# TencentARC/SEED-Story

Measured on AMD Instinct MI355X. Metric: story-steps/sec (text + 1024x1024 image), higher is better.
Workload: dtype bf16

## Files before the change

seed-story_amd/csrc/ss_attn.hip:

```cpp
#include "ss_common.h"

namespace ss {

struct AttnArgs {
    const void *q, *k, *v;
    void* out;
    int q_len, kv_len, hd, n_heads;
    int64_t q_sb, q_sh, q_ss, k_sb, k_sh, k_ss, v_sb, v_sh, v_ss, o_sb, o_sh, o_ss;
    float scale;
    int causal_br;
    int xcd_heads;
    int ragged;
    int kv_len_b[8];
};

template <typename T> struct AttnMma;
template <> struct AttnMma<bf16_t> {
    static __device__ __forceinline__ f32x4_t run(const uint4& a, const uint4& b, f32x4_t c) {
        return __builtin_amdgcn_mfma_f32_16x16x32_bf16(__builtin_bit_cast(bf16x8_t, a),
                                                       __builtin_bit_cast(bf16x8_t, b), c, 0, 0, 0);
    }
};
template <> struct AttnMma<f16_t> {
    static __device__ __forceinline__ f32x4_t run(const uint4& a, const uint4& b, f32x4_t c) {
// ... 311 lines not shown
                    }
            } else {
#pragma unroll
                for (int kb = 0; kb < NKB; ++kb)
#pragma unroll
                    for (int r = 0; r < 4; ++r) tmax = fmaxf(tmax, s[qb][kb][r]);
            }
            tmax = fmaxf(tmax, __shfl_xor(tmax, 16, 64));
            tmax = fmaxf(tmax, __shfl_xor(tmax, 32, 64));
            const float m_new = fmaxf(m_run[qb], tmax);
            const float alpha = __builtin_amdgcn_exp2f((m_run[qb] - m_new) * sl2);
            const float nm = -fmaxf(m_new, -1e29f) * sl2;
            float lsum = 0.f;
#pragma unroll
            for (int kb = 0; kb < NKB; ++kb)
#pragma unroll
                for (int r = 0; r < 4; ++r) {
                    const float p = __builtin_amdgcn_exp2f(fmaf(s[qb][kb][r], sl2, nm));
                    s[qb][kb][r] = p;
                    lsum += p;
                }
            lsum += __shfl_xor(lsum, 16, 64);
            lsum += __shfl_xor(lsum, 32, 64);
            l_run[qb] = l_run[qb] * alpha + lsum;
            m_run[qb] = m_new;
#pragma unroll
            for (int i = 0; i < NDB; ++i)
#pragma unroll
                for (int r = 0; r < 4; ++r) o[qb][i][r] *= alpha;
#pragma unroll
            for (int kp2 = 0; kp2 < NKB / 2; ++kp2) {
                float pf[8];
#pragma unroll
                for (int r = 0; r < 4; ++r) { pf[r] = s[qb][2 * kp2][r]; pf[4 + r] = s[qb][2 * kp2 + 1][r]; }
                pfrag[qb][kp2] = pack<T>(pf);
            }
        }
#pragma unroll
        for (int kp2 = 0; kp2 < NKB / 2; ++kp2) {
#pragma unroll
            for (int db = 0; db < NDB; ++db) {
                const int kr0 = (2 * kp2) * 16 + grp * 4 + (l15 >> 2);
                const int dcol = db * 16 + (l15 & 3) * 4;
                const v4s_t v0 = __builtin_amdgcn_ds_read_tr16_b64_v4i16((lds_v4s_t*)(Vb + kr0 * ROWB + dcol * 2));
                const v4s_t v1 = __builtin_amdgcn_ds_read_tr16_b64_v4i16((lds_v4s_t*)(Vb + (kr0 + 16) * ROWB + dcol * 2));
                const uint2 w0 = __builtin_bit_cast(uint2, v0), w1 = __builtin_bit_cast(uint2, v1);
                const uint4 vfrag = make_uint4(w0.x, w0.y, w1.x, w1.y);
                o[0][db] = AttnMma<T>::run(vfrag, pfrag[0][kp2], o[0][db]);
                o[1][db] = AttnMma<T>::run(vfrag, pfrag[1][kp2], o[1][db]);
            }
        }
    }

#pragma unroll
    for (int qb = 0; qb < 2; ++qb) {
        if (qi[qb] >= a.q_len) continue;
        const float inv = l_run[qb] > 0.f ? 1.0f / l_run[qb] : 0.f;
        T* op = (T*)a.out + (int64_t)b * a.o_sb + (int64_t)h * a.o_sh + (int64_t)qi[qb] * a.o_ss;
#pragma unroll
        for (int db = 0; db < NDB; ++db) {
            const int d = db * 16 + grp * 4;
            if (d + 3 < hd && ((a.o_ss | a.o_sh | a.o_sb) & 3) == 0) {
                float pk[8] = {o[qb][db][0] * inv, o[qb][db][1] * inv, o[qb][db][2] * inv, o[qb][db][3] * inv, 0, 0, 0, 0};
                const uint4 u = pack<T>(pk);
                *reinterpret_cast<uint2*>(op + d) = make_uint2(u.x, u.y);
            } else {
#pragma unroll
                for (int r = 0; r < 4; ++r)
                    if (d + r < hd) Tr<T>::st(op + d + r, o[qb][db][r] * inv);
            }
        }
    }
}
#endif

__device__ __forceinline__ float max3_asm(float a, float b, float c) {
    float r;
    asm("v_max3_f32 %0, %1, %2, %3" : "=v"(r) : "v"(a), "v"(b), "v"(c));
    return r;
}
template <typename T> struct OnesFrag;
template <> struct OnesFrag<bf16_t> { static constexpr uint32_t kPair = 0x3F803F80u; };
template <> struct OnesFrag<f16_t> { static constexpr uint32_t kPair = 0x3C003C00u; };
__device__ __forceinline__ void attn_block_of_grid(const AttnArgs& a, int& bh, int& qblk) {
    if (gridDim.y == 1 && a.xcd_heads > 0) {
        const int id = blockIdx.x, xcd = id & 7, j = id >> 3;
        const int nqb = a.xcd_heads;
        bh = (j / nqb) * 8 + xcd;
        qblk = j - (j / nqb) * nqb;
    } else {
        bh = blockIdx.y; qblk = blockIdx.x;
    }
}

template <typename T, int HD>
__device__ __forceinline__ void flash_compute_s(const char* Kb, int l15, int grp, const uint4 (&qf)[2][HD / 32],
                                                f32x4_t (&s)[2][kBKV / 16]) {
    constexpr int CPR = HD / 8, ROWB = HD * 2;
#pragma unroll
    for (int kb = 0; kb < kBKV / 16; ++kb) {
        s[0][kb] = f32x4_t{0.f, 0.f, 0.f, 0.f};
        s[1][kb] = f32x4_t{0.f, 0.f, 0.f, 0.f};
        const int r = kb * 16 + l15;
#pragma unroll
        for (int ks = 0; ks < HD / 32; ++ks) {
            const uint4 kf = *reinterpret_cast<const uint4*>(Kb + r * ROWB + (((ks * 4 + grp) ^ (r & (CPR - 1))) << 4));
            s[0][kb] = AttnMma<T>::run(kf, qf[0][ks], s[0][kb]);
            s[1][kb] = AttnMma<T>::run(kf, qf[1][ks], s[1][kb]);
        }
    }
}

template <typename T, int HD, bool VSWZ>
__global__ __launch_bounds__(256) __attribute__((amdgpu_waves_per_eu(HD <= 64 ? 3 : 2)))
void flash_attn3_kernel(const AttnArgs a) {
    constexpr int V = 8;
    constexpr int BQ2 = 128;
    constexpr int CPR = HD / V;
    constexpr int KPI = 64 / CPR;
    constexpr int NI = kBKV / KPI;
    constexpr int IPW = NI / 4;
    constexpr int ROWB = HD * 2;
    constexpr int TILE_B = kBKV * ROWB;
    constexpr int NDB = HD / 16, NKB = kBKV / 16, NKS = HD / 32;
    constexpr float THR_L2 = 8.0f;
    extern __shared__ __attribute__((aligned(16))) char smem_raw[];

    const int tid = threadIdx.x, lane = tid & 63;
    const int wid = __builtin_amdgcn_readfirstlane(tid >> 6);
    const int l15 = lane & 15, grp = lane >> 4;
    int bh, qblk;
    attn_block_of_grid(a, bh, qblk);
    const int b = bh / a.n_heads, h = bh % a.n_heads;
    const int kvl = a.ragged ? a.kv_len_b[b] : a.kv_len;
    const int q0 = qblk * BQ2;
    const int hd = a.hd;
    const T* __restrict__ qp = (const T*)a.q + (int64_t)b * a.q_sb + (int64_t)h * a.q_sh;
    const T* __restrict__ kp = (const T*)a.k + (int64_t)b * a.k_sb + (int64_t)h * a.k_sh;
    const T* __restrict__ vp = (const T*)a.v + (int64_t)b * a.v_sb + (int64_t)h * a.v_sh;
    const int shift = kvl - a.q_len;
    const T* zero = reinterpret_cast<const T*>(g_attn_zero_page);
    const uint32_t lds0 = __builtin_amdgcn_readfirstlane((uint32_t)(size_t)(lds_void2_t*)smem_raw);
    const float sl2 = a.scale * 1.4426950408889634f;
    const float thr_raw = THR_L2 / fmaxf(sl2, 1e-30f);

    int qi[2];
    uint4 qf[2][NKS];
#pragma unroll
    for (int qb = 0; qb < 2; ++qb) {
        qi[qb] = q0 + wid * 32 + qb * 16 + l15;
#pragma unroll
        for (int ks = 0; ks < NKS; ++ks) {
            const int d = ks * 32 + grp * 8;
            qf[qb][ks] = (qi[qb] < a.q_len && d < hd) ? ld16(qp + (int64_t)qi[qb] * a.q_ss + d) : make_uint4(0, 0, 0, 0);
        }
    }
    f32x4_t o[2][NDB], osum[2];
#pragma unroll
    for (int qb = 0; qb < 2; ++qb) {
        osum[qb] = f32x4_t{0.f, 0.f, 0.f, 0.f};
#pragma unroll
        for (int i = 0; i < NDB; ++i) o[qb][i] = f32x4_t{0.f, 0.f, 0.f, 0.f};
    }
    float m_run[2] = {-1e30f, -1e30f};
    const uint4 ones = make_uint4(OnesFrag<T>::kPair, OnesFrag<T>::kPair, OnesFrag<T>::kPair, OnesFrag<T>::kPair);

// ... 62 lines not shown
#pragma unroll
                for (int kb = 0; kb < NKB; ++kb)
#pragma unroll
                    for (int r = 0; r < 4; ++r) {
                        const int kg = t0 + kb * 16 + grp * 4 + r;
                        const bool ok = kg < kvl && (!a.causal_br || kg <= qi[qb] + shift);
                        s[qb][kb][r] = ok ? s[qb][kb][r] : -1e30f;
                    }
            }
            float tmax;
            asm volatile("s_nop 7\n\ts_nop 7\n\tv_max3_f32 %0, %1, %2, %3"
                         : "=v"(tmax) : "v"(s[qb][0][0]), "v"(s[qb][0][1]), "v"(s[qb][0][2]));
            tmax = max3_asm(tmax, s[qb][0][3], s[qb][1][0]);
#pragma unroll
            for (int kb = 1; kb < NKB; ++kb) {
                tmax = max3_asm(tmax, s[qb][kb][1], s[qb][kb][2]);
                if (kb + 1 < NKB) tmax = max3_asm(tmax, s[qb][kb][3], s[qb][kb + 1][0]);
                else tmax = max3_asm(tmax, s[qb][kb][3], s[qb][kb][3]);
            }
            if (__any(tmax > m_run[qb] + thr_raw)) {
                tmax = fmaxf(tmax, __shfl_xor(tmax, 16, 64));
                tmax = fmaxf(tmax, __shfl_xor(tmax, 32, 64));
                const float m_new = fmaxf(m_run[qb], tmax);
                const float alpha = __builtin_amdgcn_exp2f((m_run[qb] - m_new) * sl2);
                m_run[qb] = m_new;
#pragma unroll
                for (int i = 0; i < NDB; ++i)
#pragma unroll
                    for (int r = 0; r < 4; ++r) o[qb][i][r] *= alpha;
#pragma unroll
                for (int r = 0; r < 4; ++r) osum[qb][r] *= alpha;
            }
            const float nm = -fmaxf(m_run[qb], -1e29f) * sl2;
#pragma unroll
            for (int kp2 = 0; kp2 < NKB / 2; ++kp2) {
                float pf[8];
#pragma unroll
                for (int r = 0; r < 4; ++r) {
                    pf[r] = __builtin_amdgcn_exp2f(fmaf(s[qb][2 * kp2][r], sl2, nm));
                    pf[4 + r] = __builtin_amdgcn_exp2f(fmaf(s[qb][2 * kp2 + 1][r], sl2, nm));
                }
                pfrag[qb][kp2] = pack<T>(pf);
            }
        }
#pragma unroll
        for (int kp2 = 0; kp2 < NKB / 2; ++kp2) {
            osum[0] = AttnMma<T>::run(ones, pfrag[0][kp2], osum[0]);
            osum[1] = AttnMma<T>::run(ones, pfrag[1][kp2], osum[1]);
#pragma unroll
            for (int db = 0; db < NDB; ++db) {
                const char* vb = Vb + voff[db] + kp2 * 32 * ROWB;
                const v4s_t v0 = __builtin_amdgcn_ds_read_tr16_b64_v4i16((lds_v4s_t*)(vb));
                const v4s_t v1 = __builtin_amdgcn_ds_read_tr16_b64_v4i16((lds_v4s_t*)(vb + 16 * ROWB));
                const uint2 w0 = __builtin_bit_cast(uint2, v0), w1 = __builtin_bit_cast(uint2, v1);
                const uint4 vfrag = make_uint4(w0.x, w0.y, w1.x, w1.y);
                o[0][db] = AttnMma<T>::run(vfrag, pfrag[0][kp2], o[0][db]);
                o[1][db] = AttnMma<T>::run(vfrag, pfrag[1][kp2], o[1][db]);
            }
        }
    }

#pragma unroll
    for (int qb = 0; qb < 2; ++qb) {
        if (qi[qb] >= a.q_len) continue;
        const float l = osum[qb][0];
        const float inv = l > 0.f ? 1.0f / l : 0.f;
        T* op = (T*)a.out + (int64_t)b * a.o_sb + (int64_t)h * a.o_sh + (int64_t)qi[qb] * a.o_ss;
#pragma unroll
        for (int db = 0; db < NDB; ++db) {
            const int d = db * 16 + grp * 4;
            if (d + 3 < hd && ((a.o_ss | a.o_sh | a.o_sb) & 3) == 0) {
                float pk[8] = {o[qb][db][0] * inv, o[qb][db][1] * inv, o[qb][db][2] * inv, o[qb][db][3] * inv, 0, 0, 0, 0};
                const uint4 u = pack<T>(pk);
                *reinterpret_cast<uint2*>(op + d) = make_uint2(u.x, u.y);
            } else {
#pragma unroll
                for (int r = 0; r < 4; ++r)
                    if (d + r < hd) Tr<T>::st(op + d + r, o[qb][db][r] * inv);
            }
        }
    }
}

template <typename T, int HD, bool PIPE, int NW = 4>
__global__ __launch_bounds__(64 * NW) __attribute__((amdgpu_waves_per_eu(PIPE ? 2 : (NW >= 8 ? 4 : 3))))
void flash_attn3p_kernel(const AttnArgs a) {
    static_assert(HD == 64, "v3p: head_dim <= 64");
    static_assert(NW == 4 || NW == 8 || NW == 16, "waves per workgroup");
    constexpr int V = 8;
    constexpr int BQ2 = 32 * NW;
    constexpr int CPR = HD / V;
    constexpr int KPI = 64 / CPR;
    constexpr int NI = kBKV / KPI;
    constexpr int IPW = NI / NW > 0 ? NI / NW : 1;
    constexpr int ROWB = HD * 2;
    constexpr int TILE_B = kBKV * ROWB;
    constexpr int NDB = HD / 16, NKB = kBKV / 16, NKS = HD / 32;
    constexpr int NSTAGE = 3;
    constexpr float THR_L2 = 8.0f;
    extern __shared__ __attribute__((aligned(16))) char smem_raw[];

    const int tid = threadIdx.x, lane = tid & 63;
    const int wid = __builtin_amdgcn_readfirstlane(tid >> 6);
    const int l15 = lane & 15, grp = lane >> 4;
    int bh, qblk;
    attn_block_of_grid(a, bh, qblk);
    const int b = bh / a.n_heads, h = bh % a.n_heads;
    const int kvl = a.ragged ? a.kv_len_b[b] : a.kv_len;
    const int q0 = qblk * BQ2;
    const int hd = a.hd;
    const T* __restrict__ qp = (const T*)a.q + (int64_t)b * a.q_sb + (int64_t)h * a.q_sh;
    const T* __restrict__ kp = (const T*)a.k + (int64_t)b * a.k_sb + (int64_t)h * a.k_sh;
    const T* __restrict__ vp = (const T*)a.v + (int64_t)b * a.v_sb + (int64_t)h * a.v_sh;
    const int shift = kvl - a.q_len;
    const T* zero = reinterpret_cast<const T*>(g_attn_zero_page);
    const uint32_t lds0 = __builtin_amdgcn_readfirstlane((uint32_t)(size_t)(lds_void2_t*)smem_raw);
    const float sl2 = a.scale * 1.4426950408889634f;
    const float thr_raw = THR_L2 / fmaxf(sl2, 1e-30f);

    int qi[2];
    uint4 qf[2][NKS];
#pragma unroll
    for (int qb = 0; qb < 2; ++qb) {
        qi[qb] = q0 + wid * 32 + qb * 16 + l15;
#pragma unroll
        for (int ks = 0; ks < NKS; ++ks) {
            const int d = ks * 32 + grp * 8;
            qf[qb][ks] = (qi[qb] < a.q_len && d < hd) ? ld16(qp + (int64_t)qi[qb] * a.q_ss + d) : make_uint4(0, 0, 0, 0);
        }
    }
    f32x4_t o[2][NDB], osum[2];
#pragma unroll
    for (int qb = 0; qb < 2; ++qb) {
        osum[qb] = f32x4_t{0.f, 0.f, 0.f, 0.f};
#pragma unroll
        for (int i = 0; i < NDB; ++i) o[qb][i] = f32x4_t{0.f, 0.f, 0.f, 0.f};
    }
    float m_run[2] = {-1e30f, -1e30f};
    const uint4 ones = make_uint4(OnesFrag<T>::kPair, OnesFrag<T>::kPair, OnesFrag<T>::kPair, OnesFrag<T>::kPair);

    int kv_end = kvl;
    if (a.causal_br) {
        const int lim = q0 + BQ2 - 1 + shift + 1;
        if (lim < kv_end) kv_end = lim;
        if (kv_end < 0) kv_end = 0;
    }
    const int ntiles = (kv_end + kBKV - 1) / kBKV;
    if (ntiles == 0) {
#pragma unroll
        for (int qb = 0; qb < 2; ++qb) {
            if (qi[qb] >= a.q_len) continue;
            T* op = (T*)a.out + (int64_t)b * a.o_sb + (int64_t)h * a.o_sh + (int64_t)qi[qb] * a.o_ss;
#pragma unroll
            for (int db = 0; db < NDB; ++db)
#pragma unroll
                for (int r = 0; r < 4; ++r) {
                    const int d = db * 16 + grp * 4 + r;
                    if (d < hd) Tr<T>::st(op + d, 0.f);
                }
        }
        return;
    }

    auto vsw = [](int r) { return (r >> 1) & 3; };

    const int skey = lane / CPR, spc = lane % CPR;
    int dkey[IPW];
    const T* kbase_l[IPW];
    const T* vbase_l[IPW];
// ... 26 lines not shown
            attn_dma16(vs, __builtin_amdgcn_readfirstlane(vbase + roff));
        }
    };

    const int vrow = grp * 4 + (l15 >> 2);
    uint32_t voff[NDB];
#pragma unroll
    for (int db = 0; db < NDB; ++db) voff[db] = (uint32_t)(vrow * ROWB + ((db ^ vsw(vrow)) << 5) + (l15 & 3) * 8);

    auto compute_s = [&](int slot, f32x4_t (&s)[2][NKB]) {
        const char* Kb = smem_raw + slot * 2 * TILE_B;
        flash_compute_s<T, HD>(Kb, l15, grp, qf, s);
    };

    auto softmax_pv = [&](int t, int slot, f32x4_t (&s)[2][NKB]) {
        const char* Vb = smem_raw + slot * 2 * TILE_B + TILE_B;
        const int t0 = t * kBKV;
        uint4 pfrag[2][NKB / 2];
        const bool need_mask = a.causal_br || (t0 + kBKV > kvl);
#pragma unroll
        for (int qb = 0; qb < 2; ++qb) {
            if (need_mask) {
#pragma unroll
                for (int kb = 0; kb < NKB; ++kb)
#pragma unroll
                    for (int r = 0; r < 4; ++r) {
                        const int kg = t0 + kb * 16 + grp * 4 + r;
                        const bool ok = kg < kvl && (!a.causal_br || kg <= qi[qb] + shift);
                        s[qb][kb][r] = ok ? s[qb][kb][r] : -1e30f;
                    }
            }
            float tmax;
            asm volatile("s_nop 7\n\ts_nop 7\n\tv_max3_f32 %0, %1, %2, %3"
                         : "=v"(tmax) : "v"(s[qb][0][0]), "v"(s[qb][0][1]), "v"(s[qb][0][2]));
            tmax = max3_asm(tmax, s[qb][0][3], s[qb][1][0]);
#pragma unroll
            for (int kb = 1; kb < NKB; ++kb) {
                tmax = max3_asm(tmax, s[qb][kb][1], s[qb][kb][2]);
                if (kb + 1 < NKB) tmax = max3_asm(tmax, s[qb][kb][3], s[qb][kb + 1][0]);
                else tmax = max3_asm(tmax, s[qb][kb][3], s[qb][kb][3]);
            }
            if (__any(tmax > m_run[qb] + thr_raw)) {
                tmax = fmaxf(tmax, __shfl_xor(tmax, 16, 64));
                tmax = fmaxf(tmax, __shfl_xor(tmax, 32, 64));
                const float m_new = fmaxf(m_run[qb], tmax);
                const float alpha = __builtin_amdgcn_exp2f((m_run[qb] - m_new) * sl2);
                m_run[qb] = m_new;
#pragma unroll
                for (int i = 0; i < NDB; ++i)
#pragma unroll
                    for (int r = 0; r < 4; ++r) o[qb][i][r] *= alpha;
#pragma unroll
                for (int r = 0; r < 4; ++r) osum[qb][r] *= alpha;
            }
            const float nm = -fmaxf(m_run[qb], -1e29f) * sl2;
#pragma unroll
            for (int kp2 = 0; kp2 < NKB / 2; ++kp2) {
                float pf[8];
#pragma unroll
                for (int r = 0; r < 4; ++r) {
                    pf[r] = __builtin_amdgcn_exp2f(fmaf(s[qb][2 * kp2][r], sl2, nm));
                    pf[4 + r] = __builtin_amdgcn_exp2f(fmaf(s[qb][2 * kp2 + 1][r], sl2, nm));
                }
                pfrag[qb][kp2] = pack<T>(pf);
            }
        }
#pragma unroll
        for (int kp2 = 0; kp2 < NKB / 2; ++kp2) {
            osum[0] = AttnMma<T>::run(ones, pfrag[0][kp2], osum[0]);
            osum[1] = AttnMma<T>::run(ones, pfrag[1][kp2], osum[1]);
#pragma unroll
            for (int db = 0; db < NDB; ++db) {
                const char* vb = Vb + voff[db] + kp2 * 32 * ROWB;
                const v4s_t v0 = __builtin_amdgcn_ds_read_tr16_b64_v4i16((lds_v4s_t*)(vb));
                const v4s_t v1 = __builtin_amdgcn_ds_read_tr16_b64_v4i16((lds_v4s_t*)(vb + 16 * ROWB));
                const uint2 w0 = __builtin_bit_cast(uint2, v0), w1 = __builtin_bit_cast(uint2, v1);
                const uint4 vfrag = make_uint4(w0.x, w0.y, w1.x, w1.y);
                o[0][db] = AttnMma<T>::run(vfrag, pfrag[0][kp2], o[0][db]);
                o[1][db] = AttnMma<T>::run(vfrag, pfrag[1][kp2], o[1][db]);
            }
        }
    };

    if constexpr (!PIPE) {
        issue_tile(0, 0);
        if (1 < ntiles) issue_tile(1, 1);
        int stage = 0;
        f32x4_t sc[2][NKB];
        for (int t = 0; t < ntiles; ++t) {
            if (t + 1 < ntiles) asm volatile("s_waitcnt vmcnt(%0)" ::"n"(2 * IPW) : "memory");
            else asm volatile("s_waitcnt vmcnt(0)" ::: "memory");
            __syncthreads();
            if (t + NSTAGE - 1 < ntiles) {
                int ns = stage + NSTAGE - 1;
                if (ns >= NSTAGE) ns -= NSTAGE;
                issue_tile(t + NSTAGE - 1, ns);
            }
            compute_s(stage, sc);
            softmax_pv(t, stage, sc);
            if (++stage == NSTAGE) stage = 0;
        }
    } else {
    issue_tile(0, 0);
    if (1 < ntiles) issue_tile(1, 1);
    if (1 < ntiles) asm volatile("s_waitcnt vmcnt(%0)" ::"n"(2 * IPW) : "memory");
    else asm volatile("s_waitcnt vmcnt(0)" ::: "memory");
    __syncthreads();
    f32x4_t sA[2][NKB], sB[2][NKB];
    compute_s(0, sA);

    auto iteration = [&](int t, int slot, f32x4_t (&cur)[2][NKB], f32x4_t (&nxt)[2][NKB]) {
        const bool more = t + 1 < ntiles;
        int s1 = slot + 1; if (s1 >= NSTAGE) s1 -= NSTAGE;
        int s2 = s1 + 1;   if (s2 >= NSTAGE) s2 -= NSTAGE;
        if (more) {
            asm volatile("s_waitcnt vmcnt(0)" ::: "memory");
            __syncthreads();
            if (t + 2 < ntiles) issue_tile(t + 2, s2);
            compute_s(s1, nxt);
        }
        softmax_pv(t, slot, cur);
    };
    int t = 0, slot = 0;
    while (true) {
        iteration(t, slot, sA, sB);
        if (++t >= ntiles) break;
        if (++slot == NSTAGE) slot = 0;
        iteration(t, slot, sB, sA);
        if (++t >= ntiles) break;
        if (++slot == NSTAGE) slot = 0;
    }
    }

#pragma unroll
    for (int qb = 0; qb < 2; ++qb) {
        if (qi[qb] >= a.q_len) continue;
        const float l = osum[qb][0];
        const float inv = l > 0.f ? 1.0f / l : 0.f;
        T* op = (T*)a.out + (int64_t)b * a.o_sb + (int64_t)h * a.o_sh + (int64_t)qi[qb] * a.o_ss;
#pragma unroll
        for (int db = 0; db < NDB; ++db) {
            const int d = db * 16 + grp * 4;
            if (d + 3 < hd && ((a.o_ss | a.o_sh | a.o_sb) & 3) == 0) {
                float pk[8] = {o[qb][db][0] * inv, o[qb][db][1] * inv, o[qb][db][2] * inv, o[qb][db][3] * inv, 0, 0, 0, 0};
                const uint4 u = pack<T>(pk);
                *reinterpret_cast<uint2*>(op + d) = make_uint2(u.x, u.y);
            } else {
#pragma unroll
                for (int r = 0; r < 4; ++r)
                    if (d + r < hd) Tr<T>::st(op + d + r, o[qb][db][r] * inv);
            }
        }
    }
}

#if SS_EXPERIMENTAL
template <typename T>
__global__ __launch_bounds__(256) __attribute__((amdgpu_waves_per_eu(2)))
void cross_attn64_kernel(const AttnArgs a, int n_items, int items_per_block, int chunks_per_pair) {
    constexpr int HD = 64, NDB = 4, NKB = 4, NKS = 2;
    const int tid = threadIdx.x, lane = tid & 63;
    const int wid = __builtin_amdgcn_readfirstlane(tid >> 6);
    const int l15 = lane & 15, grp = lane >> 4;
    const float sl2 = a.scale * 1.4426950408889634f;
    const uint4 ones = make_uint4(OnesFrag<T>::kPair, OnesFrag<T>::kPair, OnesFrag<T>::kPair, OnesFrag<T>::kPair);
    const int kvl = a.kv_len;
    const bool o_vec = ((a.o_ss | a.o_sh | a.o_sb) & 3) == 0;
    int it = blockIdx.x * items_per_block;
    int it_end = it + items_per_block;
    if (it_end > n_items) it_end = n_items;
    if (it >= it_end) return;

    uint4 kf[NKB][NKS];
    uint4 vf[NKB / 2][NDB];
    int cur_pair = -1;
    auto load_q = [&](int item, uint4 (&qf)[2][NKS]) {
        const int pair = item / chunks_per_pair, chunk = item - pair * chunks_per_pair;
        const int b = pair / a.n_heads, h = pair - b * a.n_heads;
        const T* __restrict__ qp = (const T*)a.q + (int64_t)b * a.q_sb + (int64_t)h * a.q_sh;
#pragma unroll
        for (int qb = 0; qb < 2; ++qb) {
            const int qi = chunk * 128 + wid * 32 + qb * 16 + l15;
// ... 72 lines not shown
                    pf[r] = __builtin_amdgcn_exp2f(fmaf(s[qb][2 * kp2][r], sl2, nm));
                    pf[4 + r] = __builtin_amdgcn_exp2f(fmaf(s[qb][2 * kp2 + 1][r], sl2, nm));
                }
                pfrag[qb][kp2] = pack<T>(pf);
            }
        }
        f32x4_t o[2][NDB], osum[2];
#pragma unroll
        for (int qb = 0; qb < 2; ++qb) {
            osum[qb] = f32x4_t{0.f, 0.f, 0.f, 0.f};
#pragma unroll
            for (int i = 0; i < NDB; ++i) o[qb][i] = f32x4_t{0.f, 0.f, 0.f, 0.f};
        }
#pragma unroll
        for (int kp2 = 0; kp2 < NKB / 2; ++kp2) {
            osum[0] = AttnMma<T>::run(ones, pfrag[0][kp2], osum[0]);
            osum[1] = AttnMma<T>::run(ones, pfrag[1][kp2], osum[1]);
#pragma unroll
            for (int db = 0; db < NDB; ++db) {
                o[0][db] = AttnMma<T>::run(vf[kp2][db], pfrag[0][kp2], o[0][db]);
                o[1][db] = AttnMma<T>::run(vf[kp2][db], pfrag[1][kp2], o[1][db]);
            }
        }
#pragma unroll
        for (int qb = 0; qb < 2; ++qb) {
            const int qi = chunk * 128 + wid * 32 + qb * 16 + l15;
            if (qi >= a.q_len) continue;
            const float l = osum[qb][0];
            const float inv = l > 0.f ? 1.0f / l : 0.f;
            T* op = (T*)a.out + (int64_t)b * a.o_sb + (int64_t)h * a.o_sh + (int64_t)qi * a.o_ss;
#pragma unroll
            for (int db = 0; db < NDB; ++db) {
                const int d = db * 16 + grp * 4;
                if (o_vec) {
                    float pk[8] = {o[qb][db][0] * inv, o[qb][db][1] * inv, o[qb][db][2] * inv, o[qb][db][3] * inv, 0, 0, 0, 0};
                    const uint4 u = pack<T>(pk);
                    *reinterpret_cast<uint2*>(op + d) = make_uint2(u.x, u.y);
                } else {
#pragma unroll
                    for (int r = 0; r < 4; ++r) Tr<T>::st(op + d + r, o[qb][db][r] * inv);
                }
            }
        }
        if (more) {
#pragma unroll
            for (int qb = 0; qb < 2; ++qb)
#pragma unroll
                for (int ks = 0; ks < NKS; ++ks) qf[qb][ks] = qn[qb][ks];
        }
    }
}

template <typename T>
static int cross_attn64_launch(const AttnArgs& a, int64_t batch, hipStream_t s) {
    const int cpp = cdiv(a.q_len, 128);
    const int64_t n_items = batch * a.n_heads * cpp;
    static int n_cu = 0;
    if (n_cu == 0) {
        int dev = 0;
        hipDeviceProp_t p;
        if (hipGetDevice(&dev) == hipSuccess && hipGetDeviceProperties(&p, dev) == hipSuccess) n_cu = p.multiProcessorCount;
        if (n_cu <= 0) n_cu = 256;
    }
    const int64_t max_blocks = (int64_t)2 * n_cu;
    const int ipb = (int)((n_items + max_blocks - 1) / max_blocks);
    const int grid = (int)((n_items + ipb - 1) / ipb);
    hipLaunchKernelGGL((cross_attn64_kernel<T>), dim3((unsigned)grid), dim3(256), 0, s, a, (int)n_items, ipb, cpp);
    SS_LAUNCH_CHECK("cross_attn64");
    return SS_OK;
}

#endif

static dim3 flash_grid(AttnArgs& a, int nqb, int64_t bh) {
    a.xcd_heads = 0;
    if (bh % 8 == 0 && nqb > 1 && knob(K_attn_xcd)) {
        a.xcd_heads = nqb;
        return dim3((unsigned)(nqb * bh), 1);
    }
    return dim3((unsigned)nqb, (unsigned)bh);
}

template <typename T, bool PIPE>
static int flash3p_launch(const AttnArgs& a, int64_t batch, hipStream_t s) {
    const int64_t kv_tiles = a.ragged ? 3 : cdiv(a.kv_len, kBKV);
    const size_t lds = (size_t)(kv_tiles < 3 && !PIPE ? (kv_tiles < 1 ? 1 : kv_tiles) : 3) * 2 * kBKV * 64 * 2;
    const int64_t bh = batch * a.n_heads;
    const int aw = knob(K_attn_waves);
    const bool many = a.ragged || a.kv_len >= 512;
    const bool w16 = !PIPE && (aw == 16 || (aw == 0 && many && a.q_len >= 2048 && (int64_t)cdiv(a.q_len, 512) * bh >= 1024));
    const bool w8 = !PIPE && !w16 && (aw == 8 || (aw == 0 && many && a.q_len >= 512 && (int64_t)cdiv(a.q_len, 256) * bh >= 1024));
    const int nqb = cdiv(a.q_len, w16 ? 512 : w8 ? 256 : 128);
    AttnArgs a2 = a;
    const dim3 grid = flash_grid(a2, nqb, bh);
    if constexpr (!PIPE) {
        if (w16) {
            hipLaunchKernelGGL((flash_attn3p_kernel<T, 64, false, 16>), grid, dim3(1024), lds, s, a2);
            SS_LAUNCH_CHECK("flash_attn3p");
            return SS_OK;
        }
        if (w8) {
            hipLaunchKernelGGL((flash_attn3p_kernel<T, 64, false, 8>), grid, dim3(512), lds, s, a2);
            SS_LAUNCH_CHECK("flash_attn3p");
            return SS_OK;
        }
    }
    hipLaunchKernelGGL((flash_attn3p_kernel<T, 64, PIPE>), grid, dim3(256), lds, s, a2);
    SS_LAUNCH_CHECK("flash_attn3p");
    return SS_OK;
}

template <typename T, int HD, bool VSWZ>
static int flash3_launch_hd(const AttnArgs& a, int64_t batch, hipStream_t s) {
    const size_t lds = (size_t)(HD <= 64 ? 3 : 2) * 2 * kBKV * HD * 2;
    const int nqb = cdiv(a.q_len, 128);
    const int64_t bh = batch * a.n_heads;
    AttnArgs a2 = a;
    const dim3 grid = flash_grid(a2, nqb, bh);
    hipLaunchKernelGGL((flash_attn3_kernel<T, HD, VSWZ>), grid, dim3(256), lds, s, a2);
    SS_LAUNCH_CHECK("flash_attn3");
    return SS_OK;
}

#if SS_EXPERIMENTAL
template <typename T, int HD>
static int flash2_launch_hd(const AttnArgs& a, int64_t batch, hipStream_t s) {
    const size_t lds = (size_t)(HD <= 64 ? 3 : 2) * 2 * kBKV * HD * 2;
    dim3 grid((unsigned)cdiv(a.q_len, 128), (unsigned)(batch * a.n_heads));
    hipLaunchKernelGGL((flash_attn2_kernel<T, HD>), grid, dim3(256), lds, s, a);
    SS_LAUNCH_CHECK("flash_attn2");
    return SS_OK;
}
#endif

template <typename T, int HD>
static int flash_launch_hd(const AttnArgs& a, int64_t batch, hipStream_t s) {
    constexpr int V = Tr<T>::kVec;
    const size_t lds = ((size_t)kBKV * (HD + V) + (size_t)HD * (kBKV + V)) * sizeof(T);
    dim3 grid((unsigned)cdiv(a.q_len, kBQ), (unsigned)(batch * a.n_heads));
    hipLaunchKernelGGL((flash_attn_kernel<T, HD>), grid, dim3(256), lds, s, a);
    SS_LAUNCH_CHECK("flash_attn");
    return SS_OK;
}

template <typename T>
int attention_launch(const AttnArgs& a, int64_t batch, hipStream_t s) {
    constexpr int V = Tr<T>::kVec;
    SS_REQUIRE(a.hd % V == 0 && a.hd > 0 && a.hd <= 128, "attention: head_dim %d unsupported", a.hd);
    SS_REQUIRE(a.q_ss % V == 0 && a.k_ss % V == 0 && a.v_ss % V == 0 && a.q_sh % V == 0 && a.k_sh % V == 0 &&
                   a.v_sh % V == 0 && a.q_sb % V == 0 && a.k_sb % V == 0 && a.v_sb % V == 0,
               "attention: strides must be multiples of %d elements", V);
    SS_REQUIRE(!a.causal_br || a.kv_len >= a.q_len, "attention: causal needs kv_len >= q_len");
    if (a.q_len == 0 || batch == 0) return SS_OK;
    SS_REQUIRE(a.kv_len > 0, "attention: kv_len == 0");
    if constexpr (V == 8) {
        const int ver = knob(K_attn_ver);
#if SS_EXPERIMENTAL
        if (a.hd == 64 && a.kv_len <= 64 && !a.causal_br && !a.ragged && a.q_len >= 128 && ver >= 3 && knob(K_attn_cross64))
            return cross_attn64_launch<T>(a, batch, s);
#endif
        if (ver == 5 && a.q_len >= 32 && a.hd <= 64) return flash3p_launch<T, true>(a, batch, s);
        if (ver == 6 && a.q_len >= 32 && a.hd <= 64) return flash3p_launch<T, false>(a, batch, s);
        if (ver >= 3 && a.q_len >= 32) {
            if (ver == 3 || ver >= 5) {
                if (a.hd <= 64) return flash3_launch_hd<T, 64, true>(a, batch, s);
                return flash3_launch_hd<T, 128, true>(a, batch, s);
            }
            if (a.hd <= 64) return flash3_launch_hd<T, 64, false>(a, batch, s);
            return flash3_launch_hd<T, 128, false>(a, batch, s);
        }
#if SS_EXPERIMENTAL
        if (ver == 2 && a.q_len >= 32) {
            if (a.hd <= 64) return flash2_launch_hd<T, 64>(a, batch, s);
            return flash2_launch_hd<T, 128>(a, batch, s);
        }
#else
        SS_REQUIRE(ver != 2, "attention: attn_ver 2 (flash v2) is only in the EXPERIMENTAL=1 build");
#endif
    }
    if (a.hd <= 64) return flash_launch_hd<T, 64>(a, batch, s);
    return flash_launch_hd<T, 128>(a, batch, s);
}

int attention_dev(const AttnArgs& a, int64_t batch, int dtype, hipStream_t s) {
    return SS_DISPATCH(dtype, attention_launch, a, batch, s);
}

struct DecodeArgs {
    const void* q;
    const void* qkv_raw;
    void *kc, *vc;
    const void *cos_t, *sin_t;
    float* part;
    const int32_t* kv_len_dev;
    const int32_t* pos_dev;
    const int32_t* done_flag;
    int hd, n_heads, cap, nsplit;
    float scale;
    int nb, state_stride;
    int64_t q_stride, cache_stride, part_stride, out_stride;
};

template <typename T>
__global__ __launch_bounds__(256) void attn_decode_kernel(const DecodeArgs a0) {
    DecodeArgs a = a0;
    {
        const int b = blockIdx.z;
        const int64_t so = (int64_t)b * a.state_stride;
        if (a.done_flag) a.done_flag += so;
        a.kv_len_dev += so;
        if (a.pos_dev) a.pos_dev += so;
        if (a.q) a.q = (const T*)a.q + b * a.q_stride;
        if (a.qkv_raw) a.qkv_raw = (const T*)a.qkv_raw + b * a.q_stride;
        a.kc = (T*)a.kc + b * a.cache_stride;
        a.vc = (T*)a.vc + b * a.cache_stride;
        a.part += b * a.part_stride;
    }
    constexpr int V = Tr<T>::kVec;
    constexpr int KPT = 4;
    extern __shared__ __attribute__((aligned(16))) char smem_raw[];
    float* sm = reinterpret_cast<float*>(smem_raw);
    if (a.done_flag && *a.done_flag) return;
    const int h = blockIdx.x, sp = blockIdx.y, tid = threadIdx.x;
    const int hd = a.hd;
    const int LPK = hd / V, NKG = 256 / LPK;
    const int kg = tid / LPK, dl = tid % LPK, d0 = dl * V;
    const bool fused = a.qkv_raw != nullptr;
    const int n_old = *a.kv_len_dev;
    const int kv_len = n_old + (fused ? 1 : 0);
    const int chunk = (kv_len + a.nsplit - 1) / a.nsplit;
    const int k_lo = sp * chunk;
    const int k_hi = min(kv_len, k_lo + chunk);
    const T* kh = (const T*)a.kc + (int64_t)h * a.cap * hd;
    const T* vh = (const T*)a.vc + (int64_t)h * a.cap * hd;
    const int E = a.n_heads * hd;

    auto load_kv = [&](int base, uint4 (&kk)[KPT], uint4 (&vv)[KPT]) {
#pragma unroll
        for (int i = 0; i < KPT; ++i) {
            const int key = base + i * NKG;
            if (key < k_hi && !(fused && key == n_old)) {
                kk[i] = ld16(kh + (int64_t)key * hd + d0);
                vv[i] = ld16(vh + (int64_t)key * hd + d0);
            } else {
                kk[i] = make_uint4(0, 0, 0, 0);
// ... 236 lines not shown
```

seed-story_amd/csrc/ss_knobs.h:

```cpp
#pragma once
#include <limits.h>

#include <atomic>

#define SS_KNOB_LIST(X)                                                                                                              \
                                                                                                            \
    X(attn_waves, 0, "flash v3p waves per workgroup: 0 = rule by shape, 4 / 8 / 16 = force")                                         \
    X(attn_xcd, 1, "flash v3 / v3p: one XCD owns heads k, k+8, ... (flattened grid) when batch x heads is a multiple of 8")          \
    X(attn_ver, 6, "prefill attention kernel: 6 = v3p without prefetch (hd <= 64), 5 = v3p with prefetch, 3 / 4 = v3 swizzled / "    \
                   "linear V, 2 = v2 (EXPERIMENTAL build only), below = v1")                                                         \
    X(attn_cross64, 0, "EXPERIMENTAL build: contexts of <= 64 keys at head_dim 64 keep K / V in registers (cross_attn64)")           \
    X(attn_decode_nsplit, 0, "decode attention KV splits per (head, slot): 0 = 16 / slots, else rounded up to 4 / 8 / 16 / 32")      \
                                                                                                                 \
    X(gemm_f32_split, 0, "gate mode: fp32 GEMM / GEMV through split-bf16 MFMA instead of the exact fp32 FMA chain")                  \
    X(gemm_f32_split_order, 16, "gate mode grid: bands of this many N tiles walked M-fastest; 0 = plain N-fastest grid")             \
    X(gemm_f32_split_tile, 0, "gate mode tile: 0 = rule by shape, 1 = 256x128, 2 = 128x256, 3 = 128x128")                            \
    X(gemm_cfg, 0, "force one GEMM tile id for every launch (0 = tile table, then the closed-form rule)")                            \
    X(gemm_table, 1, "consult the per-shape tile table before the closed-form rule")                                                 \
    X(gemm_autotune_log, 0, "print every candidate's time while a shape is tuned")                                                   \
    X(gemm_xcd_swizzle, 8, "tile-id swizzle of the GEMM / conv grids (0 = row-major)")                                               \
    X(gemm_epi_generic, 0, "take the generic epilogue instead of the specialised ones (A/B runs)")                                   \
    X(gemm_rowstat_fallback, 0, "skip the tiles with a statistics epilogue and take the separate-kernel fallback (tests)")           \
    X(lnfold_w4, 0, "EXPERIMENTAL build: LayerNorm-folded GEMM stays on a 4-wave tile instead of the 8-wave reroute")                \
    X(gemm_splitk, 1, "split-K plan for eligible shapes in ss_gemm_splitk")                                                          \
    X(gemm_splitk_s, 0, "force the split-K count (2..8) where the workspace and K allow it; 0 = planned count")                      \
    X(gemm_splitk_swz, 0, "tile-id swizzle of the split-K grid (0 = row-major, the measured best)")                                  \
    X(gemm_fp8_cfg, 0, "force one fp8 GEMM tile id (0 = closed-form rule)")                                                          \
    X(gemm_fp8_swz, KNOB_UNSET, "tile-id swizzle of the fp8 GEMM grid; unset = 8 with 16 or more row tiles, else 0")                 \
    X(gemm_fp8_debug, 0, "print shape, tile id and swizzle of every ss_gemm_fp8 launch")                                             \
                                                                                                          \
    X(layernorm_rows_per_wave, 1, "LayerNorm wave kernel at >= 8192 rows: rows per wave (1 | 2 | 4)")                                \
                                                                                                         \
    X(llama_graph, 1, "decode tokens replay a captured graph (0 = eager launches)")                                                  \
    X(llama_done_poll, 8, "decode tokens launched between two polls of the done flags")                                              \
    X(llama_batched_attn, 1, "prefill of 2..8 equal-length slots runs one batched attention launch")                                 \
                                                                                                                 \
    X(gemv_mfma_blocks, 256, "MFMA GEMV forms: workgroups per round of 16-row tiles")                                                \
    X(gemv_mfma_generic, 0, "MFMA GEMV: the generic kernel instead of the exact-K specialisations")                                  \
    X(gemv_mfma_long, 1, "MFMA GEMV: the packed 43-step form for K = 11008")                                                         \
    X(gemv_mfma_nt, 0, "MFMA GEMV: non-temporal weight loads (measured slower)")                                                     \
    X(gemv_max_blocks, 2048, "dot-product GEMV: cap on the workgroup count")                                                         \
    X(gemv_x_reg_packs, 16, "dot-product GEMV: x stays in registers while batch x K iterations <= this many 16-byte packs")          \
    X(gemv_force_lds, 0, "dot-product GEMV: always stage x in LDS")                                                                  \
    X(gemv_nt, 1, "dot-product GEMV: non-temporal weight loads")                                                                     \
    X(gemv_mfma_min_nb, 3, "fewest sequences that take an MFMA GEMV form")                                                           \
    X(gemv_groups_per_wave, 0, "dot-product GEMV: row groups per wave; 0 = ~2.5k waves in all")                                      \
    X(gemv_split_refused, 0, "COUNTER: gate-mode GEMV launches that could not take the split form and ran as exact sweeps")          \
                                                                                   \
    X(vae_fp32, 0, "VAE decode in fp32 whatever the module dtype")                                                                   \
    X(vae_bf16, 0, "fp16 VAE modules decode in bf16 instead of fp32")                                                                \
    X(unet_graph, 1, "denoising steps replay a captured graph")                                                                      \
    X(gemm_autotune, 1, "tune unseen GEMM shapes on first use")                                                                      \
    X(img_block_logits, 1, "image-token blocks also compute the reference's (unused) per-position logits")                           \
    X(img_block_decode, KNOB_UNSET, "forced image-token blocks decode as one block; unset = the SEEDSTORY_IMG_BLOCK environment rule")                \
    X(llama_decode_w8, 0, "LlamaEngine default of decode_weights: 1 = fp8 (e4m3) weight-only decode projections")                \
    X(llama_decode_mx4, 0, "LlamaEngine default of decode_weights: 1 = MXFP4 weight-only decode projections (not with llama_decode_w8)") \
    X(llama_kv8, 0, "LlamaEngine default of kv_cache: 1 = decode attention reads an fp8 (e4m3) shadow of the KV cache")                  \
    X(llama_spec_rows, 0, "LlamaEngine default of speculate: rows (2..8) of a prompt-lookup speculative step of generate; 0 = off")

namespace ss {

constexpr int KNOB_UNSET = INT_MIN;

enum Knob : int {
#define X(name, dflt, doc) K_##name,
    SS_KNOB_LIST(X)
#undef X
    K_COUNT
};

struct KnobInfo { const char* name; int dflt; const char* doc; };
inline constexpr KnobInfo kKnobs[] = {
#define X(name, dflt, doc) {#name, dflt, doc},
    SS_KNOB_LIST(X)
#undef X
};
static_assert(sizeof(kKnobs) / sizeof(kKnobs[0]) == K_COUNT && K_COUNT == 46, "knob list and enum out of step");

extern std::atomic<int> g_knobs[K_COUNT];

inline int knob(Knob k) { return g_knobs[k].load(std::memory_order_relaxed); }
inline int knob_or(Knob k, int fallback) { const int v = knob(k); return v == KNOB_UNSET ? fallback : v; }
inline void knob_add(Knob k, int n) { g_knobs[k].fetch_add(n, std::memory_order_relaxed); }

}
```

Measured before the change: 2.465.

## Add interleaved flash-attention loop body with software-pipelined K/V LDS reads

Adds an ILV variant of the non-prefetch v3p flash-attention kernel. It double-buffers K fragment reads against the QK MFMAs using sched_group_barrier hints, and rotates a three-deep V fragment buffer across the PV MFMAs. It also precomputes the negated scaled running max so each exp2 is a single fma, and uses a reordered max tree. The variant is enabled by default for non-ragged shapes with kv_len >= 512, at the cost of more registers and more scheduling constraints.

```diff
diff --git a/seed-story_amd/csrc/ss_attn.hip b/seed-story_amd/csrc/ss_attn.hip
--- a/seed-story_amd/csrc/ss_attn.hip
+++ b/seed-story_amd/csrc/ss_attn.hip
@@ -417,6 +417,7 @@
 template <typename T> struct OnesFrag;
 template <> struct OnesFrag<bf16_t> { static constexpr uint32_t kPair = 0x3F803F80u; };
 template <> struct OnesFrag<f16_t> { static constexpr uint32_t kPair = 0x3C003C00u; };
+__device__ __forceinline__ float max3_sched(float a, float b, float c) { return __builtin_fmaxf(__builtin_fmaxf(a, b), c); }
 __device__ __forceinline__ void attn_block_of_grid(const AttnArgs& a, int& bh, int& qblk) {
     if (gridDim.y == 1 && a.xcd_heads > 0) {
         const int id = blockIdx.x, xcd = id & 7, j = id >> 3;
@@ -645,9 +646,10 @@
     }
 }
 
-template <typename T, int HD, bool PIPE, int NW = 4>
+template <typename T, int HD, bool PIPE, int NW = 4, bool ILV = false>
 __global__ __launch_bounds__(64 * NW) __attribute__((amdgpu_waves_per_eu(PIPE ? 2 : (NW >= 8 ? 4 : 3))))
 void flash_attn3p_kernel(const AttnArgs a) {
+    static_assert(!(PIPE && ILV), "the interleaved body is a form of the PIPE = false loop");
     static_assert(HD == 64, "v3p: head_dim <= 64");
     static_assert(NW == 4 || NW == 8 || NW == 16, "waves per workgroup");
     constexpr int V = 8;
@@ -840,6 +842,130 @@
         }
     };
 
+    auto compute_s_ahead = [&](int slot, f32x4_t (&s)[2][NKB]) {
+        const char* Kb = smem_raw + slot * 2 * TILE_B;
+        auto kread = [&](int kb, int ks) {
+            const int r = kb * 16 + l15;
+            return *reinterpret_cast<const uint4*>(Kb + r * ROWB + (((ks * 4 + grp) ^ (r & (CPR - 1))) << 4));
+        };
+        uint4 kf[2][NKS];
+#pragma unroll
+        for (int ks = 0; ks < NKS; ++ks) kf[0][ks] = kread(0, ks);
+#pragma unroll
+        for (int kb = 0; kb < NKB; ++kb) {
+            if (kb + 1 < NKB) {
+#pragma unroll
+                for (int ks = 0; ks < NKS; ++ks) kf[(kb + 1) & 1][ks] = kread(kb + 1, ks);
+            }
+            s[0][kb] = f32x4_t{0.f, 0.f, 0.f, 0.f};
+            s[1][kb] = f32x4_t{0.f, 0.f, 0.f, 0.f};
+#pragma unroll
+            for (int ks = 0; ks < NKS; ++ks) {
+                s[0][kb] = AttnMma<T>::run(kf[kb & 1][ks], qf[0][ks], s[0][kb]);
+                s[1][kb] = AttnMma<T>::run(kf[kb & 1][ks], qf[1][ks], s[1][kb]);
+            }
+        }
+        __builtin_amdgcn_sched_group_barrier(0x100, 2 * NKS, 0);
+#pragma unroll
+        for (int kb = 0; kb < NKB; ++kb) {
+            __builtin_amdgcn_sched_group_barrier(0x008, 2 * NKS, 0);
+            if (kb + 2 < NKB) __builtin_amdgcn_sched_group_barrier(0x100, NKS, 0);
+        }
+    };
+
+    float nm_run[2] = {-fmaxf(m_run[0], -1e29f) * sl2, -fmaxf(m_run[1], -1e29f) * sl2};
+
+    auto softmax_pv_ilv = [&](int t, int slot, f32x4_t (&s)[2][NKB]) {
+        const char* Vb = smem_raw + slot * 2 * TILE_B + TILE_B;
+        const int t0 = t * kBKV;
+        uint4 pfrag[2][NKB / 2];
+        const bool need_mask = a.causal_br || (t0 + kBKV > kvl);
+        if (need_mask) {
+#pragma unroll
+            for (int qb = 0; qb < 2; ++qb)
+#pragma unroll
+                for (int kb = 0; kb < NKB; ++kb)
+#pragma unroll
+                    for (int r = 0; r < 4; ++r) {
+                        const int kg = t0 + kb * 16 + grp * 4 + r;
+                        const bool ok = kg < kvl && (!a.causal_br || kg <= qi[qb] + shift);
+                        s[qb][kb][r] = ok ? s[qb][kb][r] : -1e30f;
+                    }
+        }
+        float tmax[2], ca[2], cb[2];
+#pragma unroll
+        for (int qb = 0; qb < 2; ++qb) ca[qb] = max3_sched(s[qb][0][0], s[qb][0][1], s[qb][0][2]);
+#pragma unroll
+        for (int qb = 0; qb < 2; ++qb) ca[qb] = max3_sched(ca[qb], s[qb][0][3], s[qb][1][0]);
+#pragma unroll
+        for (int qb = 0; qb < 2; ++qb) cb[qb] = max3_sched(s[qb][2][1], s[qb][2][2], s[qb][2][3]);
+#pragma unroll
+        for (int qb = 0; qb < 2; ++qb) ca[qb] = max3_sched(ca[qb], s[qb][1][1], s[qb][1][2]);
+#pragma unroll
+        for (int qb = 0; qb < 2; ++qb) cb[qb] = max3_sched(cb[qb], s[qb][3][0], s[qb][3][1]);
+#pragma unroll
+        for (int qb = 0; qb < 2; ++qb) ca[qb] = max3_sched(ca[qb], s[qb][1][3], s[qb][2][0]);
+#pragma unroll
+        for (int qb = 0; qb < 2; ++qb) cb[qb] = max3_sched(cb[qb], s[qb][3][2], s[qb][3][3]);
+#pragma unroll
+        for (int qb = 0; qb < 2; ++qb) tmax[qb] = max3_sched(ca[qb], cb[qb], s[qb][0][0]);
+        if (__any(tmax[0] > m_run[0] + thr_raw || tmax[1] > m_run[1] + thr_raw)) {
+#pragma unroll
+            for (int qb = 0; qb < 2; ++qb) {
+                if (__any(tmax[qb] > m_run[qb] + thr_raw)) {
+                    float tm = tmax[qb];
+                    tm = fmaxf(tm, __shfl_xor(tm, 16, 64));
+                    tm = fmaxf(tm, __shfl_xor(tm, 32, 64));
+                    const float m_new = fmaxf(m_run[qb], tm);
+                    const float alpha = __builtin_amdgcn_exp2f((m_run[qb] - m_new) * sl2);
+                    m_run[qb] = m_new;
+                    nm_run[qb] = -fmaxf(m_new, -1e29f) * sl2;
+#pragma unroll
+                    for (int i = 0; i < NDB; ++i)
+#pragma unroll
+                        for (int r = 0; r < 4; ++r) o[qb][i][r] *= alpha;
+#pragma unroll
+                    for (int r = 0; r < 4; ++r) osum[qb][r] *= alpha;
+                }
+            }
+        }
+#pragma unroll
+        for (int qb = 0; qb < 2; ++qb)
+#pragma unroll
+            for (int kp2 = 0; kp2 < NKB / 2; ++kp2) {
+                float pf[8];
+#pragma unroll
+                for (int r = 0; r < 4; ++r) {
+                    pf[r] = __builtin_amdgcn_exp2f(fmaf(s[qb][2 * kp2][r], sl2, nm_run[qb]));
+                    pf[4 + r] = __builtin_amdgcn_exp2f(fmaf(s[qb][2 * kp2 + 1][r], sl2, nm_run[qb]));
+                }
+                pfrag[qb][kp2] = pack<T>(pf);
+            }
+        auto vread = [&](int kp2, int db) {
+            const char* vb = Vb + voff[db] + kp2 * 32 * ROWB;
+            const v4s_t v0 = __builtin_amdgcn_ds_read_tr16_b64_v4i16((lds_v4s_t*)(vb));
+            const v4s_t v1 = __builtin_amdgcn_ds_read_tr16_b64_v4i16((lds_v4s_t*)(vb + 16 * ROWB));
+            const uint2 w0 = __builtin_bit_cast(uint2, v0), w1 = __builtin_bit_cast(uint2, v1);
+            return make_uint4(w0.x, w0.y, w1.x, w1.y);
+        };
+        uint4 vf[3];
+        vf[0] = vread(0, 0);
+        vf[1] = vread(0, 1);
+        __builtin_amdgcn_sched_barrier(0);
+#pragma unroll
+        for (int i = 0; i < 2 * NDB; ++i) {
+            const int kp2 = i / NDB, db = i % NDB;
+            if (i + 2 < 2 * NDB) vf[(i + 2) % 3] = vread((i + 2) / NDB, (i + 2) % NDB);
+            if (db == 0) {
+                osum[0] = AttnMma<T>::run(ones, pfrag[0][kp2], osum[0]);
+                osum[1] = AttnMma<T>::run(ones, pfrag[1][kp2], osum[1]);
+            }
+            o[0][db] = AttnMma<T>::run(vf[i % 3], pfrag[0][kp2], o[0][db]);
+            o[1][db] = AttnMma<T>::run(vf[i % 3], pfrag[1][kp2], o[1][db]);
+            __builtin_amdgcn_sched_barrier(0);
+        }
+    };
+
     if constexpr (!PIPE) {
         issue_tile(0, 0);
         if (1 < ntiles) issue_tile(1, 1);
@@ -854,8 +980,13 @@
                 if (ns >= NSTAGE) ns -= NSTAGE;
                 issue_tile(t + NSTAGE - 1, ns);
             }
-            compute_s(stage, sc);
-            softmax_pv(t, stage, sc);
+            if constexpr (ILV) {
+                compute_s_ahead(stage, sc);
+                softmax_pv_ilv(t, stage, sc);
+            } else {
+                compute_s(stage, sc);
+                softmax_pv(t, stage, sc);
+            }
             if (++stage == NSTAGE) stage = 0;
         }
     } else {
@@ -1094,7 +1225,7 @@
 }
 
 template <typename T, bool PIPE>
-static int flash3p_launch(const AttnArgs& a, int64_t batch, hipStream_t s) {
+static int flash3p_launch(const AttnArgs& a, int64_t batch, hipStream_t s, bool ilv_all = false) {
     const int64_t kv_tiles = a.ragged ? 3 : cdiv(a.kv_len, kBKV);
     const size_t lds = (size_t)(kv_tiles < 3 && !PIPE ? (kv_tiles < 1 ? 1 : kv_tiles) : 3) * 2 * kBKV * 64 * 2;
     const int64_t bh = batch * a.n_heads;
@@ -1106,6 +1237,14 @@
     AttnArgs a2 = a;
     const dim3 grid = flash_grid(a2, nqb, bh);
     if constexpr (!PIPE) {
+        const bool ilv = ilv_all || (knob(K_attn_ilv) != 0 && !a.ragged && a.kv_len >= 512);
+        if (ilv) {
+            if (w16) hipLaunchKernelGGL((flash_attn3p_kernel<T, 64, false, 16, true>), grid, dim3(1024), lds, s, a2);
+            else if (w8) hipLaunchKernelGGL((flash_attn3p_kernel<T, 64, false, 8, true>), grid, dim3(512), lds, s, a2);
+            else hipLaunchKernelGGL((flash_attn3p_kernel<T, 64, false, 4, true>), grid, dim3(256), lds, s, a2);
+            SS_LAUNCH_CHECK("flash_attn3p");
+            return SS_OK;
+        }
         if (w16) {
             hipLaunchKernelGGL((flash_attn3p_kernel<T, 64, false, 16>), grid, dim3(1024), lds, s, a2);
             SS_LAUNCH_CHECK("flash_attn3p");
@@ -1173,6 +1312,7 @@
 #endif
         if (ver == 5 && a.q_len >= 32 && a.hd <= 64) return flash3p_launch<T, true>(a, batch, s);
         if (ver == 6 && a.q_len >= 32 && a.hd <= 64) return flash3p_launch<T, false>(a, batch, s);
+        if (ver == 7 && a.q_len >= 32 && a.hd <= 64) return flash3p_launch<T, false>(a, batch, s, true);
         if (ver >= 3 && a.q_len >= 32) {
             if (ver == 3 || ver >= 5) {
                 if (a.hd <= 64) return flash3_launch_hd<T, 64, true>(a, batch, s);
diff --git a/seed-story_amd/csrc/ss_knobs.h b/seed-story_amd/csrc/ss_knobs.h
--- a/seed-story_amd/csrc/ss_knobs.h
+++ b/seed-story_amd/csrc/ss_knobs.h
@@ -7,8 +7,9 @@
                                                                                                             \
     X(attn_waves, 0, "flash v3p waves per workgroup: 0 = rule by shape, 4 / 8 / 16 = force")                                         \
     X(attn_xcd, 1, "flash v3 / v3p: one XCD owns heads k, k+8, ... (flattened grid) when batch x heads is a multiple of 8")          \
-    X(attn_ver, 6, "prefill attention kernel: 6 = v3p without prefetch (hd <= 64), 5 = v3p with prefetch, 3 / 4 = v3 swizzled / "    \
-                   "linear V, 2 = v2 (EXPERIMENTAL build only), below = v1")                                                         \
+    X(attn_ver, 6, "prefill attention kernel: 6 = v3p without prefetch (hd <= 64), 7 = 6 with the interleaved loop body on every "   \
+                   "launch, 5 = v3p with prefetch, 3 / 4 = v3 swizzled / linear V, 2 = v2 (EXPERIMENTAL build only), below = v1")    \
+    X(attn_ilv, 1, "attn_ver 6: 1 = the shape classes where the attn_ver 7 loop body measured a win take it, 0 = never")            \
     X(attn_cross64, 0, "EXPERIMENTAL build: contexts of <= 64 keys at head_dim 64 keep K / V in registers (cross_attn64)")           \
     X(attn_decode_nsplit, 0, "decode attention KV splits per (head, slot): 0 = 16 / slots, else rounded up to 4 / 8 / 16 / 32")      \
                                                                                                                  \
@@ -75,7 +76,7 @@
     SS_KNOB_LIST(X)
 #undef X
 };
-static_assert(sizeof(kKnobs) / sizeof(kKnobs[0]) == K_COUNT && K_COUNT == 46, "knob list and enum out of step");
+static_assert(sizeof(kKnobs) / sizeof(kKnobs[0]) == K_COUNT && K_COUNT == 47, "knob list and enum out of step");
 
 extern std::atomic<int> g_knobs[K_COUNT];
 
```

Result: no change. 2.481 (median of 6 runs) (+0.6%).
